# bastienjacquet/CudaDepthMapIntegration

Measured on AMD Instinct MI355X. Metric: Gvoxel-projections/s, higher is better.
Workload: dtype f64

## Files before the change

### cudadepthmapintegration_amd/build.py

```python
from __future__ import annotations

import os
import re
import shutil
import subprocess
from concurrent.futures import ThreadPoolExecutor

_HERE = os.path.dirname(os.path.abspath(__file__))
ROOT = os.path.dirname(_HERE)
CSRC = os.path.join(_HERE, "csrc")
OBJ_DIR = os.path.join(ROOT, "build", "obj")
LIB_PATH = os.path.join(CSRC, "libdmi_hip.so")

SOURCES = ["fusion_kernels.hip", "fusion_tile.hip", "fusion_classify.hip", "coloration_kernels.hip", "mesh_depth_render.hip", "grid_post.hip", "point_smooth.hip", "isosurface.hip", "isosurface_components.hip", "isosurface_smooth.hip", "isosurface_decimate.hip", "isosurface_holes.hip", "isosurface_support.hip", "depth_consistency.hip", "depth_speckle.hip", "depth_holes.hip", "depth_smooth.hip", "scene_bounds.hip", "depth_points.hip", "depth_points_thin.hip", "depth_points_radius.hip", "dmi_capi.hip", "dmi_capi_views.hip", "dmi_capi_fuse.hip", "dmi_capi_mesh.hip", "dmi_capi_color.hip", "dmi_capi_consistency.hip", "dmi_capi_speckle.hip", "dmi_capi_holes.hip", "dmi_capi_smooth.hip", "dmi_capi_bounds.hip", "dmi_capi_points_thin.hip", "dmi_capi_points_radius.hip", "view_set_kernels.hip", "dmi_capi_viewset.hip", "dmi_multi.hip", "host/recon_host.cpp", "host/vti_reader.cpp", "host/vtp_reader.cpp", "host/recon_cli.cpp", "host/color_cli.cpp", "host/dmi_host_capi.cpp"]
HEADERS = ["fusion_kernels.h", "view_records.h", "fusion_launch_rules.h", "fusion_device.h", "dmi_buffer.h", "dmi_depth_call.h", "dmi_mesh_stage.h", "dmi_context.h", "dmi_color_context.h", "coloration_kernels.h", "mesh_depth_render.h", "depth_consistency.h", "depth_speckle.h", "depth_speckle_rules.h", "depth_holes.h", "depth_holes_rules.h", "depth_smooth.h", "depth_smooth_rules.h", "union_find_device.h", "scene_bounds.h", "scene_bounds_rules.h", "depth_points.h", "depth_points_rules.h", "depth_points_thin.h", "depth_points_thin_rules.h", "depth_points_radius.h", "depth_points_radius_rules.h", "dmi_view_set.h", "view_set_kernels.h", "view_set_rules.h", "point_smooth_rules.h", "rounded_quotient.h", "fusion_tile_acc.inc", "isosurface_table.inc", os.path.join("host", "recon_host.h"),
           os.path.join("host", "vtk_xml_data.h"), os.path.join("host", "vti_reader.h"), os.path.join("host", "vtp_reader.h"),
           os.path.join("host", "recon_cli.h"), os.path.join("host", "color_cli.h"), os.path.join("host", "fan_triangulate.h"),
           os.path.join("..", "..", "include", "dmi.h"), os.path.join("..", "..", "include", "dmi_host.h")]
CLI_MAINS = ["recon_cli_main.cpp", "color_cli_main.cpp"]

COMMON_FLAGS = ["-O3", "-std=c++17", "-fPIC", "-ffp-contract=off", "-fno-fast-math", "-Wall", "-Wno-unused-function",
                "-Wno-inline-asm", "-Wno-pass-failed"]
HIP_FLAGS = ["--offload-arch=gfx950", "-mllvm", "-disable-promote-alloca-to-vector", "-Xoffload-linker", "--discard-all"]
OPTIONAL_LLVM_FLAGS = ["-amdgpu-use-amdgpu-trackers=1"]
# ... 83 lines not shown
        return True
    t = os.path.getmtime(target)
    return any(os.path.getmtime(d) > t for d in deps)


LIB_OVERRIDE = os.environ.get("DMI_LIB_OVERRIDE")
if LIB_OVERRIDE:
    LIB_PATH = os.path.abspath(LIB_OVERRIDE)


def source_digest(files=None) -> str:
    import hashlib

    h = hashlib.sha256()
    h.update(" ".join(COMMON_FLAGS + HIP_FLAGS).encode())
    if files is None:
        files = [os.path.join(CSRC, s) for s in _sources()] + _headers() + [os.path.join(CSRC, "host", m) for m in CLI_MAINS]
    for f in files:
        h.update(os.path.relpath(f, CSRC).encode())
        with open(f, "rb") as fh:
            h.update(fh.read())
    return h.hexdigest()


def _digest_path() -> str:
    return LIB_PATH + ".digest"


def needs_build() -> bool:
    if LIB_OVERRIDE:
        return False
    if not os.path.exists(LIB_PATH):
        return True
    if os.path.exists(_digest_path()):
        with open(_digest_path()) as fh:
            return fh.read().strip() != source_digest()
    deps = [os.path.join(CSRC, s) for s in _sources()] + _headers()
    return _stale(LIB_PATH, deps)


ACC_BASES = {8: 64, 7: 72, 6: 80, 5: 96}


def audit_accumulator_registers(asm_text: str) -> tuple[int, list[str]]:
    import re

    bad: list[str] = []
    checked = 0
    for body in re.split(r"\n(?=_ZN3dmi\S*fuse_tile_kernel\S*:)", asm_text):
        m = re.match(r"(_ZN3dmi\S*fuse_tile_kernelI\w+):", body)
        if not m:
            continue
        name = m.group(1)
        tpl = re.search(r"fuse_tile_kernelI\w\wLi(\d+)ELi(\d)ELi(\d)ELi(\d)ELi(\d)ELb([01])", name)
        tk, minw = int(tpl.group(1)), int(tpl.group(4))
        base = ACC_BASES.get(minw, 128)
        code = body[: body.find("s_endpgm")]
        in_asm = False
        scc_from_asm = False
        for line in code.splitlines():
            if "#ASMSTART" in line:
                in_asm = True
                continue
            if "#ASMEND" in line:
                in_asm = False
                continue
            op = line.split()[0] if line.split() else ""
            if in_asm:
                if op.startswith("s_and_saveexec"):
                    scc_from_asm = True
            elif op.startswith("s_"):
                if scc_from_asm and re.match(r"s_(cbranch_scc|cselect|cmov|addc|subb)", op):
                    bad.append(f"{name}: {op} reads the SCC an asm statement's s_and_saveexec_b64 wrote: {line.strip()}")
                if not re.match(r"s_(mov|movk|load|buffer_load|waitcnt|nop|branch|cbranch|cselect|cmov|getpc|setpc|swappc|sleep|barrier|endpgm)", op):
                    scc_from_asm = False
            elif line.rstrip().endswith(":") and not line.startswith((" ", "\t")):
                scc_from_asm = False
            if in_asm or not re.match(r"\s+(v_|global_|buffer_|ds_|scratch_|flat_)", line):
                continue
            regs = [int(x) for x in re.findall(r"\bv(\d+)\b", line)]
            for a, b in re.findall(r"\bv\[(\d+):(\d+)\]", line):
                regs += [int(a), int(b)]
            if any(r >= base for r in regs):
                bad.append(f"{name}: compiler instruction touches the accumulator file (base v{base}): {line.strip()}")
        d = re.search(r"\.amdhsa_kernel " + re.escape(name) + r"\b.*?\.amdhsa_next_free_vgpr (\d+)", asm_text, re.S)
        if not d:
            bad.append(f"{name}: no kernel descriptor found")
        elif int(d.group(1)) < base + 2 * tk:
            bad.append(f"{name}: descriptor allocates {d.group(1)} VGPRs, the accumulators need {base + 2 * tk}")
        checked += 1
    if checked == 0:
        bad.append("no fuse_tile_kernel instantiation found in the assembly")
    return checked, bad


def scratch_sizes(asm_text: str) -> dict:
    import re

    out = {}
    for m in re.finditer(r"\.amdhsa_kernel (_ZN3dmi\S*fuse_tile_kernel\S*)\b(.*?)\.end_amdhsa_kernel", asm_text, re.S):
        size = re.search(r"\.amdhsa_private_segment_fixed_size (\d+)", m.group(2))
        out[m.group(1)] = int(size.group(1)) if size else 0
    return out


def lds_sizes(asm_text: str) -> dict:
    out = {}
    for m in re.finditer(r"\.amdhsa_kernel (_ZN3dmi\S*fuse_tile_kernel\S*)\b(.*?)\.end_amdhsa_kernel", asm_text, re.S):
        size = re.search(r"\.amdhsa_group_segment_fixed_size (\d+)", m.group(2))
        out[m.group(1)] = int(size.group(1)) if size else 0
    return out


def wait_state_counts(asm_text: str) -> dict:
    import re

    out = {}
    for m in re.finditer(r"^(_ZN3dmi\S*fuse_tile_kernel\S*):.*?\.end_amdhsa_kernel", asm_text, re.S | re.M):
        out[m.group(1)] = len(re.findall(r"^\s*s_nop\b", m.group(0), re.M))
    return out


def _audit_digest() -> str:
    return source_digest([os.path.join(CSRC, "fusion_tile.hip")] + _headers())


def audit_is_current() -> bool:
    import json

    marker = os.path.join(OBJ_DIR, "acc_audit.json")
    try:
        with open(marker) as fh:
            return json.load(fh).get("digest") == _audit_digest()
    except (OSError, ValueError):
        return False


def run_accumulator_audit(verbose: bool = False) -> int:
    import json
    import tempfile

    hipcc = hipcc_path()
    with tempfile.TemporaryDirectory() as tmp:
        out = os.path.join(tmp, "fusion_tile.s")
        cmd = [hipcc] + COMMON_FLAGS + HIP_FLAGS + ["--cuda-device-only", "-S", os.path.join(CSRC, "fusion_tile.hip"), "-o", out]
        if verbose:
            print(" ".join(cmd), flush=True)
        subprocess.check_call(cmd)
        with open(out) as fh:
            text = fh.read()
    checked, bad = audit_accumulator_registers(text)
    scratch = scratch_sizes(text)
    nops = wait_state_counts(text)
    lds = lds_sizes(text)
    table = {}
    for name, size in scratch.items():
        m = re.search(r"fuse_tile_kernelI(\w)(\w)Li(\d+)ELi(\d)ELi(\d)ELi(\d)ELi(\d)ELb([01])ELb([01])ELb([01])ELb([01])ELb([01])(?:ELb([01]))?E", name)
        if not m:
            continue
        depth, grid, tk, wx, wy, minw, group, count, rot, genk, stay, win, zf = m.groups()
        key = f"depth={depth} grid={grid} tk={tk} waves={wx}x{wy} count={count} rot={rot} genk={genk} stay={stay} win={win} zf={zf or 0}"
        production = depth == "f" and count == "0" and genk == "0" and wx == "1" and wy == "1"
        limit = None if not production else ((16 if "-DDMI_TUNING" in COMMON_FLAGS else 0) if tk == "16" else 48)
        table[key] = {"scratch_bytes_per_lane": size, "production": production, "limit": limit, "s_nop": nops.get(name),
                      "lds_bytes_per_workgroup": lds.get(name, 0)}
        if limit is not None and size > limit:
            bad.append(f"{name}: {size} bytes of scratch memory per lane in a production instantiation (limit {limit})")
        waves_per_cu = 4 * (4 if tk == "16" else 5)
        if production and lds.get(name, 0) * waves_per_cu > 160 * 1024:
            bad.append(f"{name}: {lds[name]} bytes of LDS per one-wave workgroup: {waves_per_cu} of them do not fit a CU's 160 KB")
    if bad:
        raise RuntimeError("accumulator-register audit of fusion_tile.hip FAILED (a toolchain change broke the hidden "
                           "register file; results would be silently wrong):\n  " + "\n  ".join(bad[:20]))
    version = subprocess.run([hipcc, "--version"], capture_output=True, text=True).stdout.strip().splitlines()
    os.makedirs(OBJ_DIR, exist_ok=True)
    with open(os.path.join(OBJ_DIR, "acc_audit.json"), "w") as fh:
        json.dump({"instantiations": checked, "violations": 0, "hipcc": version[:2], "digest": _audit_digest(),
                   "scratch_bytes_per_lane": {"max": max(scratch.values()) if scratch else None,
                                              "instantiations_with_scratch": sum(1 for v in scratch.values() if v),
                                              "production_max": max([v["scratch_bytes_per_lane"] for v in table.values() if v["production"]] or [0])},
                   "instantiation_table": table}, fh, indent=1)
    if verbose:
        print(f"accumulator audit: {checked} fuse_tile_kernel instantiations clean ({version[0] if version else 'hipcc'})", flush=True)
    return checked


def _record(mode: str) -> None:
    import json
    import time

    try:
        os.makedirs(OBJ_DIR, exist_ok=True)
        with open(os.path.join(OBJ_DIR, "build_record.json"), "w") as fh:
            json.dump({"mode": mode, "library": os.path.relpath(LIB_PATH, ROOT), "digest": source_digest(), "time": time.time(),
                       "flags": COMMON_FLAGS + HIP_FLAGS}, fh)
    except OSError:
        pass


def build(force: bool = False, verbose: bool = False) -> str:
    if not force and not needs_build():
        _record("up_to_date: the library's digest file names the present sources and flags; nothing compiled")
        return LIB_PATH
    hipcc = hipcc_path()
    os.makedirs(OBJ_DIR, exist_ok=True)
    headers = _headers()
    digest = source_digest()
    if not force and os.path.exists(LIB_PATH) and os.path.exists(_digest_path()):
        srcs = [os.path.join(CSRC, s) for s in _sources()]
        if not any(_stale(_obj(s), [p] + headers) for s, p in zip(_sources(), srcs)):
# ... 67 lines not shown
```

### cudadepthmapintegration_amd/csrc/fusion_tile.hip

```cpp
#include <stdlib.h>

#include <algorithm>
#include <type_traits>

#include "fusion_kernels.h"
#include "fusion_device.h"

#ifndef DMI_T1_CHAINS
#define DMI_T1_CHAINS 4
#endif
#ifndef DMI_T1_COLUMN_CHAINS
#define DMI_T1_COLUMN_CHAINS 2
#endif
#if !defined(DMI_TUNING) && (defined(DMI_EXP_SKIP_WINDOW_VIEWS) || defined(DMI_EXP_SAME_REC) || defined(DMI_EXP_NO_WINDOW_LOADS) || \
                             defined(DMI_EXP_NO_LANE_MARGIN))
#error "a DMI_EXP_* switch that changes results was defined without DMI_TUNING"
#endif

namespace dmi {

int tile_shape_index(int variant);

namespace {

constexpr int kLX = 8, kLY = 8;
typedef unsigned long long mask_t;


#include "fusion_tile_acc.inc"

__device__ __forceinline__ void or_where(uint32_t &bits, mask_t m, uint32_t bit ) {
  mask_t saved;
  asm("s_and_saveexec_b64 %1, %2\n\tv_or_b32 %0, %3, %0\n\ts_mov_b64 exec, %1" : "+v"(bits), "=&s"(saved) : "s"(m), "s"(bit) : "scc");
}

__device__ __forceinline__ mask_t ballot(bool p) { return __builtin_amdgcn_ballot_w64(p); }

template <typename P>
__device__ __forceinline__ P launder(P p) {
  asm volatile("" : "+s"(p));
  return p;
}

__device__ __forceinline__ int pinned_word(int x) {
  asm volatile("" : "+v"(x));
  return __builtin_amdgcn_readfirstlane(x);
}
template <typename T>
__device__ __forceinline__ const T *pinned_ptr(const T *p) {
  const uintptr_t v = reinterpret_cast<uintptr_t>(p);
  const uint32_t lo = (uint32_t)pinned_word((int)(uint32_t)v), hi = (uint32_t)pinned_word((int)(uint32_t)(v >> 32));
  return reinterpret_cast<const T *>(((uintptr_t)hi << 32) | lo);
}
__device__ __forceinline__ double pinned(double x) {
  return __hiloint2double(pinned_word(__double2hiint(x)), pinned_word(__double2loint(x)));
}

__device__ __forceinline__ int cvt_saturating(double x) {
  int r;
  asm("v_cvt_i32_f64 %0, %1" : "=v"(r) : "v"(x));
  return r;
}

typedef float f32x2 __attribute__((ext_vector_type(2)));
__device__ __forceinline__ f32x2 pk_fma_lo0_vs(f32x2 a, f32x2 b, unsigned long long c_bits) {
  f32x2 d;
// ... 154 lines not shown
  static __device__ __forceinline__ raw_t load_at(__amdgpu_buffer_rsrc_t rsrc, unsigned byte_offset) {
    typedef unsigned int u32x2 __attribute__((ext_vector_type(2)));
    const u32x2 raw = __builtin_amdgcn_raw_buffer_load_b64(rsrc, (int)byte_offset, 0, 0);
    return __hiloint2double((int)raw.y, (int)raw.x);
  }
  static __device__ __forceinline__ void opaque(raw_t &d) { asm("" : "+v"(d)); }
  static __device__ __forceinline__ bool is_sentinel(raw_t d) { return d == -1.0; }
  static __device__ __forceinline__ raw_t sentinel() { return -1.0; }
  static __device__ __forceinline__ raw_t minus_inf() { return -__builtin_inf(); }
  static __device__ __forceinline__ double widen(raw_t d) { return d; }
};

template <typename DepthT>
__device__ __forceinline__ bool tile_exact(const FuseArgs *__restrict__ fa, int m, __amdgpu_buffer_rsrc_t rsrc, int i,
                                           int j, int k, double &val) {
  double g[12], rt[12], kk[12];
  const MapRec *maps = cload(&fa->maps);
#pragma unroll
  for (int q = 0; q < 12; ++q) {
    g[q] = cload(&fa->g[q]);
    rt[q] = cload(&maps[m].rt[q]);
    kk[q] = cload(&maps[m].k[q]);
  }
  const int W = cload(&fa->W), H = cload(&fa->H);
  const double gx = cload(&fa->ox) + (i + 0.5) * cload(&fa->sx);
  const double gy = cload(&fa->oy) + (j + 0.5) * cload(&fa->sy);
  const double gz = cload(&fa->oz) + ((k + cload(&fa->kz0)) + 0.5) * cload(&fa->sz);
  const double wx = row4(g + 0, gx, gy, gz);
  const double wy = row4(g + 4, gx, gy, gz);
  const double wz = row4(g + 8, gx, gy, gz);
  const double cx = row4(rt + 0, wx, wy, wz);
  const double cy = row4(rt + 4, wx, wy, wz);
  const double cz = row4(rt + 8, wx, wy, wz);
  const double hx = row4(kk + 0, cx, cy, cz);
  const double hy = row4(kk + 4, cx, cy, cz);
  const double hz = row4(kk + 8, cx, cy, cz);
  int px = 0, py = 0;
  if (!pixel_exact(hx, hy, hz, W, H, px, py)) return false;
  const typename DepthLoad<DepthT>::raw_t d = DepthLoad<DepthT>::load(rsrc, (unsigned)(W * py + px));
  if (DepthLoad<DepthT>::is_sentinel(d)) return false;
  val = ray_potential_values(cload(&fa->thick), cload(&fa->delta), cload(&fa->rho_pos), cload(&fa->rho_neg), cload(&fa->rho_zero),
                             cload(&fa->slope), cload(&fa->free_space), cz, DepthLoad<DepthT>::widen(d));
  return true;
}

constexpr int acc_base(int minw) { return minw >= 8 ? 64 : minw == 7 ? 72 : minw == 6 ? 80 : minw == 5 ? 96 : 128; }

template <typename DepthT, typename GridT, int TK, int WX, int WY, int MINW, int GROUP, bool COUNT, bool ROT = false, bool GENK = false,
          bool STAY = (WX * WY == 1), bool WIN = false, bool ZF = false>
__global__ __launch_bounds__(64 * WX * WY, MINW) void fuse_tile_kernel(const TileArgs a) {
  typedef DepthLoad<DepthT> DL;
  static_assert(!WIN || (DMI_TIER1 != 0 && !GENK && !COUNT && WX * WY == 1), "the window column is a tier-1 column without hit counters");
  static_assert(!ZF || !COUNT, "hit counters take every view singly");
  typedef const TileArgs __attribute__((address_space(4))) *kernarg_t;
  const kernarg_t ka = (kernarg_t)__builtin_amdgcn_kernarg_segment_ptr();
  (void)a;
#define KA(f) (ka->f)
#define KC(f) (launder(ka)->f)
#define KFRESH() launder(ka)
  constexpr int BASE = acc_base(MINW);
  constexpr int kGroup = GROUP;
  typedef double czvec __attribute__((ext_vector_type(GROUP)));
  typedef double czvec4 __attribute__((ext_vector_type(4)));
  const int first_map = KA(first_map);
  const int m_end = first_map + KA(n_maps);
  double delta = KA(delta), thick = KA(thick), free_space = KA(free_space), rho_pos = KA(rho_pos), slope = KA(slope);
  int keep_zero_adds = ZF ? 0 : (KA(behind_mask) == 0 ? 1 : 0);
  free_space = pinned(free_space), rho_pos = pinned(rho_pos);
  if constexpr (!ZF) keep_zero_adds = pinned_word(keep_zero_adds);
  asm volatile("" : "+v"(delta), "+v"(thick), "+v"(slope));
  unsigned vW = (unsigned)KA(W), vH = (unsigned)KA(H);
  asm("" : "+v"(vW));
  asm("" : "+v"(vH));
  [[maybe_unused]] const double Wd = pinned((double)KA(W));
  constexpr bool T1 = DMI_TIER1 != 0 && !GENK;
  [[maybe_unused]] const float Wf = __int_as_float(pinned_word(__float_as_int((float)KA(W))));
  [[maybe_unused]] const unsigned row_bytes = (unsigned)pinned_word((int)((unsigned)KA(W) * (unsigned)sizeof(DepthT)));
  [[maybe_unused]] unsigned pix_adj = ((unsigned)(KA(W) * (KA(H) / 2) + KA(W) / 2) - 0x400000u * (unsigned)KA(W)) * (unsigned)sizeof(DepthT) - 0x4B400000u;
  constexpr bool kConstantsInVgprs = TK >= 16;
  if constexpr (T1 && kConstantsInVgprs) asm volatile("" : "+v"(pix_adj));
  if constexpr (T1 && !kConstantsInVgprs) pix_adj = (unsigned)pinned_word((int)pix_adj);
  double tiny = 0x1p-20;
  asm volatile("" : "+v"(tiny));
  const int lane = threadIdx.x & 63;
  const int w = __builtin_amdgcn_readfirstlane(threadIdx.x >> 6);

  constexpr bool PERSIST = STAY && WX * WY == 1;
  const int b = blockIdx.x;
  int q = b >> 3;
  int helped = 0;
#define DMI_NEXT_BRICK \
  {                    \
    if (PERSIST)       \
      continue;        \
    else               \
      return;          \
  }
  for (;;) {
  const kernarg_t kb = KFRESH();
  typedef int i32x8 __attribute__((ext_vector_type(8)));
  const i32x8 head0 = *reinterpret_cast<const i32x8 __attribute__((address_space(4))) *>(kb);
  const i32x8 head1 = *(reinterpret_cast<const i32x8 __attribute__((address_space(4))) *>(kb) + 1);
  const int32_t *const p_order = kb->order, *const p_levels = kb->order_levels, *const p_n_order = kb->n_order;
  const int kflags = kb->flags;
  const int xq = (b + helped) & 7;
  if constexpr (PERSIST) {
// ... 619 lines not shown
    if constexpr (T1) {
      hx = __builtin_fma(cload(&rec->cpx), wxf,
                         __builtin_fma(cload(&rec->cpy), wyf, __builtin_fma(cload(&rec->cpz), wzf, cload(&rec->cp0))));
      hy = __builtin_fma(cload(&rec->cqx), wxf,
                         __builtin_fma(cload(&rec->cqy), wyf, __builtin_fma(cload(&rec->cqz), wzf, cload(&rec->cq0))));
      const float czf = (float)cz_first;
      H0.x = (float)hx;
      H0.y = (float)hy;
      C0.x = czf;
      const float hb = max_abs(H0.x, H0.y) + cload(&rec->t1_hspan);
      float e1 = cload(&rec->t1_e1);
      if (cload(&rec->t1_ok) == 2) e1 = t1_lane_margin<TK>(czf, cload(&rec->t1_dcz), hb, e1, cload(&rec->t1_b));
      C0.y = __builtin_fmaf(czf, cload(&rec->t1_c1), -__builtin_fmaf(hb, cload(&rec->t1_erel), e1));
      DH.x = cload(&rec->t1_dhx);
      DH.y = cload(&rec->t1_dhy);
      DC.x = cload(&rec->t1_dcz);
      DC.y = cload(&rec->t1_dthr);
      asm volatile("" : "+v"(DH), "+v"(DC));
    } else if constexpr (!ROT) {
      hx = __builtin_fma(cload(&rec->px), wx,
                         __builtin_fma(cload(&rec->py), wy, __builtin_fma(cload(&rec->pz), wz0, cload(&rec->p0))));
      hy = __builtin_fma(cload(&rec->qx), wx,
                         __builtin_fma(cload(&rec->qy), wy, __builtin_fma(cload(&rec->qz), wz0, cload(&rec->q0))));
    }
    [[maybe_unused]] const double dhx = T1 ? 0.0 : cload(&rec->dhx), dhy = T1 ? 0.0 : cload(&rec->dhy), errk = T1 ? 0.0 : cload(&rec->errk);
    [[maybe_unused]] double hz = 0, dhz = 0, errz = 0;
    if constexpr (GENK) {
      dhz = cload(&rec->dhz);
      errz = cload(&rec->errz);
      if constexpr (!ROT) {
        hz = __builtin_fma(cload(&rec->sx), wx, __builtin_fma(cload(&rec->sy), wy, __builtin_fma(cload(&rec->sz), wz0, cload(&rec->s0))));
        if (!lane_ok) hz = -__builtin_inf();
      }
    }

    [[maybe_unused]] auto rot_cz = [&](int kk) __attribute__((always_inline)) -> double {
      if (kk >= kcount) return -__builtin_inf();
      const kernarg_t kr = KFRESH();
      const TileMapRec *rr = kr->tile_maps + m;
      const czvec4 b = cload(reinterpret_cast<const czvec4 *>(kr->cz_table + (int64_t)(k0 + kk) * 4));
      const double wxk = (wx + b[0]) + kr->g[3], wyk = (wy + b[1]) + kr->g[7], wzk = (wz0 + b[2]) + kr->g[11];
      return ((cload(&rr->rz0) * wxk + cload(&rr->rz1) * wyk) + cload(&kr->maps[m].rt[10]) * wzk) + sz;
    };

    uint32_t undecided = 0;
    uint32_t und_kk = 0;
    uint32_t map_hits = 0;

    auto column = [&](auto interior_tag, auto surface_tag, auto free_tag) __attribute__((always_inline)) {
      constexpr bool INTERIOR = decltype(interior_tag)::value;
      constexpr bool FREEONLY = decltype(free_tag)::value;
      constexpr bool SURFACE = decltype(surface_tag)::value;
      constexpr bool UNMASKED = INTERIOR && !COUNT;
      [[maybe_unused]] int cxc = 0, cyc = 0;
      [[maybe_unused]] unsigned bias_x = 0, bias_y = 0;
      if constexpr (T1 && !INTERIOR) {
        cxc = KC(W) >> 1;
        cyc = KC(H) >> 1;
        bias_x = 0x4B400000u - (unsigned)cxc;
        bias_y = 0x4B400000u - (unsigned)cyc;
        if constexpr (kConstantsInVgprs) asm volatile("" : "+v"(bias_x), "+v"(bias_y));
      }
      constexpr bool VMAP = T1 && FREEONLY;
      const __amdgpu_buffer_rsrc_t rsrc =
          __builtin_amdgcn_make_buffer_rsrc(const_cast<void *>(cload(&rec->depth)), (short)0, KC(depth_bytes), 0x00020000);
      mask_t m_lane_ok = m_lane_ok_brick;
      asm volatile("" : "+s"(m_lane_ok));
      [[maybe_unused]] __amdgpu_buffer_rsrc_t vrsrc = rsrc;
      [[maybe_unused]] float v_c0 = 0.f, v_w8 = 0.f;
      [[maybe_unused]] int v_base = 0;
      if constexpr (VMAP) {
        vrsrc = __builtin_amdgcn_make_buffer_rsrc(const_cast<uint8_t *>(cload(&rec->valid)), (short)0, cload(&rec->vm_bytes), 0x00020000);
        v_c0 = cload(&rec->vm_c0);
        v_w8 = cload(&rec->vm_w8);
        v_base = cload(&rec->vm_base);
      }
  #pragma unroll
      for (int g0 = 0; g0 < TK; g0 += kGroup) {
        double czg[kGroup];
        typename DL::raw_t dg[kGroup];
        [[maybe_unused]] unsigned short vg[kGroup];
        if constexpr (!ROT && !(T1 && FREEONLY)) {
          const czvec ctg = cload(reinterpret_cast<const czvec *>(ct + g0));
  #pragma unroll
          for (int q = 0; q < kGroup; ++q) czg[q] = (sz + ctg[q]) + rz3;
          __builtin_amdgcn_sched_barrier(0);
        }
        if constexpr (ROT && T1 && !FREEONLY) {
          const double c20 = cload(&rec->rz0), c21 = cload(&rec->rz1), c22 = cload(&kv->maps[m].rt[10]);
  #pragma unroll
          for (int q = 0; q < kGroup; ++q) {
            const int kk = g0 + q;
            czg[q] = -__builtin_inf();
            if (kk < kcount) {
              const czvec4 b = cload(reinterpret_cast<const czvec4 *>(kv->cz_table + (int64_t)(k0 + kk) * 4));
              const double wxk = (wx + b[0]) + KA(g)[3], wyk = (wy + b[1]) + KA(g)[7], wzk = (wz0 + b[2]) + KA(g)[11];
              czg[q] = ((c20 * wxk + c21 * wyk) + c22 * wzk) + sz;
            }
          }
        }
        constexpr int kChain = T1 && TK >= 16 ? DMI_T1_COLUMN_CHAINS : 1;
        static_assert(kGroup % kChain == 0, "whole chains per group");
  #pragma unroll
        for (int q0 = 0; q0 < kGroup; q0 += kChain) {
        [[maybe_unused]] f32x2 rpm_c[kChain], rp_c[kChain];
        [[maybe_unused]] float mx_c[kChain], thr_c[kChain];
        if constexpr (T1) {
          f32x2 h[kChain], cth[kChain], rr[kChain], t[kChain];
          const unsigned long long magic2 = 0x4B4000004B400000ull;
  #pragma unroll
          for (int u = 0; u < kChain; ++u) {
            const int kk = g0 + q0 + u;
            cth[u] = kk > 0 ? ordered::pk_fma_s((unsigned long long)(unsigned)__float_as_int((float)kk), DC, C0) : C0;
          }
  #pragma unroll
          for (int u = 0; u < kChain; ++u) {
            const int kk = g0 + q0 + u;
            h[u] = kk > 0 ? ordered::pk_fma_s((unsigned long long)(unsigned)__float_as_int((float)kk), DH, H0) : H0;
          }
  #pragma unroll
          for (int u = 0; u < kChain; ++u) rr[u].x = ordered::rcp(cth[u].x);
  #pragma unroll
          for (int u = 0; u < kChain; ++u) rpm_c[u] = ordered::pk_fma_lo_s(h[u], rr[u], magic2);
  #pragma unroll
          for (int u = 0; u < kChain; ++u) rp_c[u] = ordered::pk_sub_s(rpm_c[u], magic2);
  #pragma unroll
          for (int u = 0; u < kChain; ++u) t[u] = ordered::pk_fnma_lo(rp_c[u], cth[u], h[u]);
  #pragma unroll
          for (int u = 0; u < kChain; ++u) {
            mx_c[u] = ordered::max_abs(t[u].x, t[u].y);
            thr_c[u] = cth[u].y;
          }
        }
  #pragma unroll
        for (int qc = 0; qc < kChain; ++qc) {
          const int q = q0 + qc;
          const int kk = g0 + q;
          if constexpr (!UNMASKED) dg[q] = DL::sentinel();
          if constexpr (T1) {
            const f32x2 rpm = rpm_c[qc], rp = rp_c[qc];
            unsigned pix;
            if constexpr (VMAP) {
              const float yt = __builtin_rintf(__builtin_fmaf(rp.y, 0.125f, v_c0));
              pix = (unsigned)(cvt_i32_f32(__builtin_fmaf(yt, v_w8, __builtin_fmaf(rp.x, 8.0f, rp.y))) + v_base);
            } else {
              pix = __umul24((unsigned)__float_as_int(rpm.y), row_bytes) +
                    scaled_column_bits<sizeof(DepthT)>(rp.x) + pix_adj;
            }
            const mask_t m_p1 = ballot(mx_c[qc] < thr_c[qc]);
            mask_t m_in, m_und;
            [[maybe_unused]] mask_t m_front = 0;
            if constexpr (INTERIOR) {
              m_in = m_p1 & m_lane_ok;
              m_und = m_lane_ok & ~m_p1;
            } else {
              m_front = ballot(!(czg[q] < 0.0));
              const unsigned px1 = (unsigned)__float_as_int(rpm.x) - bias_x, py1 = (unsigned)__float_as_int(rpm.y) - bias_y;
              m_in = m_front & m_p1 & ballot((unsigned)px1 < vW) & ballot((unsigned)py1 < vH);
              m_und = m_front & ~m_p1;
            }
            if (m_und) {
              const double kd = (double)kk;
              const double hxk = __builtin_fma(kd, cload(&rec->cdhx), hx), hyk = __builtin_fma(kd, cload(&rec->cdhy), hy);
              double cz2;
              if constexpr (FREEONLY)
                cz2 = ROT ? rot_cz(kk) : (sz + cload(ct + kk)) + rz3;
              else
                cz2 = czg[q];
              const double r0 = __builtin_amdgcn_rcp(cz2);
              const double e0 = __builtin_fma(-cz2, r0, 1.0);
              const double r = __builtin_fma(r0, e0, r0);
              const double ua2 = hxk * r, va2 = hyk * r;
              const double ru2 = __builtin_rint(ua2), rv2 = __builtin_rint(va2);
              const double fu = ua2 - ru2, fv = va2 - rv2;
              const double chk = __builtin_fma(cload(&rec->cerrk), r, __builtin_fmax(__builtin_fabs(fu), __builtin_fabs(fv)));
              const mask_t m_p2 = ballot(chk < 0.5) & ballot(__builtin_fabs(e0) < tiny) & m_und;
              unsigned pix2;
              if constexpr (VMAP) {
                const double yt2 = __builtin_rint(__builtin_fma(rv2, 0.125, (double)v_c0));
                pix2 = (unsigned)(cvt_saturating(__builtin_fma(yt2, (double)v_w8, __builtin_fma(ru2, 8.0, rv2))) + v_base);
              } else {
                pix2 = (unsigned)(cvt_saturating(__builtin_fma(rv2, Wd, ru2)) + (KC(W) * (KC(H) >> 1) + (KC(W) >> 1))) * (unsigned)sizeof(DepthT);
              }
              if (__builtin_amdgcn_inverse_ballot_w64(m_p2)) pix = pix2;
              if constexpr (INTERIOR) {
                m_in |= m_p2;
              } else {
                const int px2 = cvt_saturating(ru2) + cxc, py2 = cvt_saturating(rv2) + cyc;
                m_in |= m_p2 & ballot((unsigned)px2 < vW) & ballot((unsigned)py2 < vH);
              }
              m_und &= ~m_p2;
            }
            if constexpr (VMAP && UNMASKED) {
              vg[q] = __builtin_amdgcn_raw_buffer_load_b8(vrsrc, (int)pix, 0, 0);
              if (m_und) {
                or_where(undecided, m_und, 1u << kk);
                und_kk |= 1u << kk;
                if (__builtin_amdgcn_inverse_ballot_w64(m_und)) vg[q] = 0;
              }
            } else if constexpr (UNMASKED) {
              dg[q] = DL::load_at(rsrc, pix);
              if (m_und) {
                or_where(undecided, m_und, 1u << kk);
                und_kk |= 1u << kk;
                if (__builtin_amdgcn_inverse_ballot_w64(m_und)) dg[q] = SURFACE ? DL::minus_inf() : DL::sentinel();
              }
            } else {
              if (m_und) {
                or_where(undecided, m_und, 1u << kk);
                und_kk |= 1u << kk;
              }
              if (__builtin_amdgcn_inverse_ballot_w64(m_in)) dg[q] = DL::load_at(rsrc, pix);
            }
            continue;
          }
          if constexpr (ROT) {
            if (kk >= kcount) continue;
            const czvec4 b = cload(reinterpret_cast<const czvec4 *>(kv->cz_table + (int64_t)(k0 + kk) * 4));
// ... 15 lines not shown
              if constexpr (GENK) hz += dhz;
            }
          } else {
            if constexpr (GENK) {
              if (kk >= kcount) continue;
            }
            if (kk > 0) {
              hx += dhx;
              hy += dhy;
              if constexpr (GENK) hz += dhz;
            }
          }
          const double cz = czg[q];
          const double hdiv = GENK ? hz : cz;
          const double r0 = __builtin_amdgcn_rcp(hdiv);
          const double e0 = __builtin_fma(-hdiv, r0, 1.0);
          const double r = __builtin_fma(r0, e0, r0);
          const double ua = hx * r, va = hy * r;
          const double ru = __builtin_rint(ua), rv = __builtin_rint(va);
          const double fu = ua - ru, fv = va - rv;
          const double chk = __builtin_fma(errk, r, __builtin_fmax(__builtin_fabs(fu), __builtin_fabs(fv)));
          const mask_t m_proven = ballot(chk < 0.5) & ballot(__builtin_fabs(e0) < tiny);
          mask_t m_in, m_und;
          [[maybe_unused]] mask_t m_proven_front = ~0ull;
          if constexpr (INTERIOR) {
            m_in = m_proven & m_lane_ok;
            m_und = m_lane_ok & ~m_proven;
          } else {
            const mask_t m_front = GENK ? ballot(!(hz < -errz)) : ballot(!(cz < 0.0));
            if constexpr (GENK) m_proven_front = ballot(hz > errz);
            m_in = m_front & m_proven & m_proven_front;
            m_und = m_front & ~(m_proven & m_proven_front);
          }
          if constexpr (UNMASKED) {
            dg[q] = DL::load(rsrc, (unsigned)cvt_saturating(__builtin_fma(rv, Wd, ru)));
            if (m_und) {
              or_where(undecided, m_und, 1u << kk);
              und_kk |= 1u << kk;
              if (__builtin_amdgcn_inverse_ballot_w64(m_und)) dg[q] = SURFACE ? DL::minus_inf() : DL::sentinel();
            }
          } else {
            const int px = cvt_saturating(ru), py = cvt_saturating(rv);
            if constexpr (!INTERIOR)
              m_in &= ballot((unsigned)px < vW) & ballot((unsigned)py < vH);
            if (m_und) {
              or_where(undecided, m_und, 1u << kk);
              und_kk |= 1u << kk;
            }
            if (__builtin_amdgcn_inverse_ballot_w64(m_in))
              dg[q] = DL::load(rsrc, __umul24((unsigned)py, vW) + (unsigned)px);
          }
        }
        }
  #pragma unroll
        for (int q = 0; q < kGroup; ++q) {
          const int kk = g0 + q;
          if constexpr (VMAP) {
            static_assert(kValidByte == 10, "((1 << 10) - 1) << 20 == 0x3ff00000");
            unsigned one_or_zero_hi;
            asm("v_bfm_b32 %0, %1, 20" : "=v"(one_or_zero_hi) : "v"(__builtin_bit_cast(_Float16, vg[q])));
            acc_fma_vs<BASE, TK>(kk, __hiloint2double((int)one_or_zero_hi, 0), free_space);
            continue;
          }
          const typename DL::raw_t d = dg[q];
          if constexpr (ZF && !FREEONLY) {
            if constexpr (std::is_same<DepthT, double>::value) {
              if constexpr (SURFACE) acc_potential_all_f64<BASE, TK>(kk, d, czg[q], delta, thick, slope, free_space, rho_pos);
              else acc_potential_f64<BASE, TK>(kk, d, czg[q], delta, thick, slope, free_space, rho_pos);
            } else {
              if constexpr (SURFACE) acc_potential_all_f32<BASE, TK>(kk, d, czg[q], delta, thick, slope, free_space, rho_pos);
              else acc_potential_f32<BASE, TK>(kk, d, czg[q], delta, thick, slope, free_space, rho_pos);
            }
            continue;
          }
          const mask_t m_hit = SURFACE ? ~0ull : ballot(!DL::is_sentinel(d));
          if constexpr (FREEONLY) {
            acc_add_s<BASE, TK>(kk, m_hit, free_space);
            continue;
          }
          if (SURFACE || m_hit) {
            const double diff = czg[q] - DL::widen(d);
            const mask_t m_front_far = ballot(diff < -delta);
            const mask_t m_behind_far = ballot(diff > delta);
            acc_add_s<BASE, TK>(kk, m_hit & m_front_far, free_space);
            if (!SURFACE && keep_zero_adds) acc_add_zero<BASE, TK>(kk, m_hit & m_behind_far);
            const mask_t m_near = m_hit & ~(m_front_far | m_behind_far);
            {
              if (m_near) {
                const int rh = __double2hiint(rho_pos) ^ (__double2hiint(diff) & (int)0x80000000);
                const double near = __builtin_fabs(diff) > thick ? __hiloint2double(rh, __double2loint(rho_pos)) : slope * diff;
                acc_add_v<BASE, TK>(kk, m_near, near);
              }
            }
            if (COUNT) {
              nh[kk] += __builtin_amdgcn_inverse_ballot_w64(m_hit) ? 1u : 0u;
              map_hits += (uint32_t)__popcll(m_hit);
            }
          }
        }
      }
    };
    const bool interior = kcount == TK && (cbyte & 0x1fu) >= ((unsigned)MIXED_NAN_DEPTH << 2) && !(kv->flags & TILE_FLAG_NO_INTERIOR);
    if (interior) {
      if constexpr (!COUNT) {
        if ((cbyte & 0x1fu) == ((unsigned)MIXED_FREE_OR_NODEPTH << 2 | BRICK_MIXED))
          column(std::true_type{}, std::false_type{}, std::true_type{});
#ifndef DMI_EXP_NO_SURFACE_COLUMN
        else if ((cbyte & 0x1fu) == ((unsigned)MIXED_NEAR_SURFACE << 2 | BRICK_MIXED) && !keep_zero_adds)
          column(std::true_type{}, std::true_type{}, std::false_type{});
// ... 120 lines not shown
  constexpr bool one_wave = WX * WY == 1;
  constexpr bool rare = std::is_same<DepthT, double>::value || GENK;
  static_assert(!WIN || (one_wave && !rare), "window launches are production launches");
  const int per_round = 8 * a.xcd_run_wg;
  unsigned blocks = (unsigned)((a.super_x * a.super_y * a.super_z * 32 + 32 + per_round - 1) / per_round * per_round);
  const dim3 block(64 * WX * WY);
  const bool zf = a.behind_mask != 0 && !cfg.count_hits;
  if (WIN && !zf) return hipErrorInvalidValue;
  bool stay = true;
  if constexpr (one_wave && !rare) {
    const int64_t voxels = (int64_t)a.super_x * a.super_y * a.super_z * 32 * 64 * TK;
    stay = (cfg.variant & VAR_PERSISTENT_ALWAYS) ? true
           : (cfg.variant & VAR_PERSISTENT_NEVER) ? false
           : (cfg.variant & VAR_NO_BRICK_CLASSES) ? true
           : cfg.holes ? (a.n_maps >= 48 && voxels >= (int64_t(1) << 25))
                       : (a.n_maps >= kPersistentMinViews && voxels >= (int64_t(1) << 27));
  }
  auto launch = [&](auto kernel, bool persistent, auto which) {
    unsigned n = blocks;
    if (persistent && one_wave) {
      static const unsigned resident = resident_workgroups(kernel, 64);
      n = std::min(n, resident);
    }
    (void)which;
    hipLaunchKernelGGL(kernel, dim3(n), block, 0, s, a);
    return hipGetLastError();
  };
  typedef std::integral_constant<int, 0> counted_t;
  typedef std::integral_constant<int, 1> per_brick_t;
  typedef std::integral_constant<int, 2> persistent_t;
  typedef std::integral_constant<int, 3> general_t;
  if constexpr (!WIN) {
    if (cfg.count_hits) return launch(fuse_tile_kernel<DepthT, GridT, TK, WX, WY, MINW, GROUP, true, ROT, GENK>, true, counted_t{});
  }
  if constexpr (one_wave && !rare) {
    if (zf) {
      if (!stay) return launch(fuse_tile_kernel<DepthT, GridT, TK, WX, WY, MINW, GROUP, false, ROT, GENK, false, WIN, true>, false, per_brick_t{});
      return launch(fuse_tile_kernel<DepthT, GridT, TK, WX, WY, MINW, GROUP, false, ROT, GENK, true, WIN, true>, true, persistent_t{});
    }
  }
  if constexpr (!WIN) return launch(fuse_tile_kernel<DepthT, GridT, TK, WX, WY, MINW, GROUP, false, ROT, GENK>, true, general_t{});
  return hipErrorInvalidValue;
}

int effective_shape(int variant, bool depth_is_f64, bool rotated, bool general_k = false) {
  int shape = tile_shape_index(variant);
#ifndef DMI_TUNING
  shape = (shape == 1 || shape == 3 || shape == 4 || shape == 7) ? 7 : 0;
#endif
  if (general_k || depth_is_f64) return 0;
  return (rotated && shape != 7) ? 0 : shape;
}

template <typename DepthT, typename GridT, int TK, int MINW, bool ROT>
hipError_t launch_win(const TileArgs &a, const FuseConfig &cfg, hipStream_t s) {
  if constexpr (DMI_TIER1 != 0 && std::is_same<DepthT, float>::value)
    return launch_shape<DepthT, GridT, TK, 1, 1, MINW, 8, ROT, false, true>(a, cfg, s);
  else
    return hipErrorInvalidValue;
}

template <typename DepthT, typename GridT>
hipError_t launch_types(const TileArgs &a, const FuseConfig &cfg, hipStream_t s) {
  constexpr bool f32_depth = std::is_same<DepthT, float>::value;
  const int shape = effective_shape(cfg.variant, !f32_depth, a.rotated != 0, cfg.general_k != 0);
  const bool win = DMI_TIER1 != 0 && std::is_same<DepthT, float>::value && a.win_origin != nullptr && !cfg.count_hits && !cfg.general_k &&
                   a.behind_mask != 0;
#ifdef DMI_FAST_BUILD
  if (win) {
    if (shape == 7) return launch_win<DepthT, GridT, 8, 6, false>(a, cfg, s);
    return launch_win<DepthT, GridT, 16, 5, false>(a, cfg, s);
  }
  if constexpr (f32_depth) {
    if (shape == 7) return launch_shape<DepthT, GridT, 8, 1, 1, 6, 8>(a, cfg, s);
  }
  return launch_shape<DepthT, GridT, 16, 1, 1, 5, 8>(a, cfg, s);
#else
  if (cfg.general_k) {
    if (a.rotated) return launch_shape<DepthT, GridT, 16, 1, 1, 5, 8, true, true>(a, cfg, s);
    return launch_shape<DepthT, GridT, 16, 1, 1, 5, 8, false, true>(a, cfg, s);
  }
  if (a.rotated) {
    if (win) {
      if (shape == 7) return launch_win<DepthT, GridT, 8, 6, true>(a, cfg, s);
      return launch_win<DepthT, GridT, 16, 5, true>(a, cfg, s);
    }
    if constexpr (f32_depth) {
      if (shape == 7) return launch_shape<DepthT, GridT, 8, 1, 1, 6, 8, true>(a, cfg, s);
    }
    return launch_shape<DepthT, GridT, 16, 1, 1, 5, 8, true>(a, cfg, s);
  }
#ifdef DMI_TUNING
  if constexpr (std::is_same<DepthT, float>::value) {
    switch (shape) {
      case 1: return launch_shape<DepthT, GridT, 8, 2, 2, 6, 8>(a, cfg, s);
      case 2: return launch_shape<DepthT, GridT, 16, 2, 2, 5, 8>(a, cfg, s);
      case 3: return launch_shape<DepthT, GridT, 8, 2, 2, 6, 4>(a, cfg, s);
      case 4: return launch_shape<DepthT, GridT, 8, 2, 2, 7, 8>(a, cfg, s);
      case 5: return launch_shape<DepthT, GridT, 16, 2, 2, 5, 4>(a, cfg, s);
      case 6: return launch_shape<DepthT, GridT, 16, 2, 2, 6, 2>(a, cfg, s);
      default: break;
    }
  }
#endif
  if (win && (shape == 7 || shape == 0)) {
    if (shape == 7) return launch_win<DepthT, GridT, 8, 6, false>(a, cfg, s);
    return launch_win<DepthT, GridT, 16, 5, false>(a, cfg, s);
  }
  if constexpr (f32_depth) {
    if (shape == 7) return launch_shape<DepthT, GridT, 8, 1, 1, 6, 8>(a, cfg, s);
  }
  return launch_shape<DepthT, GridT, 16, 1, 1, 5, 8>(a, cfg, s);
#endif
}

}

int tile_shape_index(int variant) { return (variant & VAR_TILE_SHAPE_MASK) >> VAR_TILE_SHAPE_SHIFT; }

TileShape tile_shape(int variant, bool depth_is_f64, bool rotated, bool general_k) {
  switch (effective_shape(variant, depth_is_f64, rotated, general_k)) {
    case 0: return TileShape{16, 1, 1};
    case 7: return TileShape{8, 1, 1};
    case 1:
    case 3:
    case 4: return TileShape{8, 2, 2};
    default: return TileShape{16, 2, 2};
  }
}

#ifdef DMI_TUNING
__global__ __launch_bounds__(256) void remap_classes_kernel(uint8_t *classes, int64_t n, uint32_t table) {
  for (int64_t i = (int64_t)blockIdx.x * blockDim.x + threadIdx.x; i < n; i += (int64_t)gridDim.x * blockDim.x) {
    const uint8_t b = classes[i];
    classes[i] = (uint8_t)((table >> (8 * (b & 3))) & 0xff);
  }
}
#endif

hipError_t launch_fuse_tiled(const TileArgs &a, const MapRec *maps_dev, const FuseConfig &cfg, const PyramidDesc &pyramid,
                             uint8_t *order_scratch, uint8_t *coarse_classes, hipEvent_t before_main_kernel,
                             hipStream_t stream) {
  if (a.n_maps <= 0) return hipSuccess;
  hipError_t e = hipSuccess;
  if (cfg.variant & VAR_NO_BRICK_CLASSES) {
    const int64_t entries = a.rotated ? a.kpad : (int64_t)a.kpad * a.n_maps;
    hipLaunchKernelGGL(launch_tables_kernel, dim3((unsigned)std::min<int64_t>((entries + 255) / 256, 4096)), dim3(256), 0, stream, a, maps_dev);
    e = hipGetLastError();
    if (e != hipSuccess) return e;
  }
  if (!(cfg.variant & VAR_NO_BRICK_CLASSES)) {
    const TileShape sh = tile_shape(cfg.variant, cfg.depth_is_f64 != 0, a.rotated != 0, cfg.general_k != 0);
    e = launch_classify_bricks(a, maps_dev, pyramid, sh.tk, const_cast<uint8_t *>(a.classes), coarse_classes, cfg.general_k, stream);
    if (e != hipSuccess) return e;
    e = launch_window_origins(a, maps_dev, sh.tk, const_cast<uint8_t *>(a.classes), cfg.general_k, stream);
    if (e != hipSuccess) return e;
#ifdef DMI_TUNING
    if (const char *env = getenv("DMI_DEBUG_CLASS_REMAP")) {
      const int64_t n = (int64_t)a.wbricks_x * a.wbricks_y * a.bricks_z * (int64_t)a.class_pitch;
      hipLaunchKernelGGL(remap_classes_kernel, dim3(4096), dim3(256), 0, stream, const_cast<uint8_t *>(a.classes), n,
                         (uint32_t)strtoul(env, nullptr, 0));
    }
#endif
    if (a.order) {
      e = launch_order_bricks(a, sh.wx, sh.wy, order_scratch, const_cast<int *>(a.order), const_cast<int *>(a.n_order), stream);
// ... 19 lines not shown
```

Baseline: 3193.

## Issue a whole 16-voxel column of depth loads per group, forming c.z late

For TK=16 tier-1 kernels on f32 depth, the load group grows from 8 to 16 so more depth loads are in flight before use. To keep register pressure in check, the per-voxel camera z values are no longer precomputed for the whole group. They are recomputed on demand in phase A and loaded in batches of four in phase B. The build audit regexes now accept a two-digit GROUP template argument. This risks higher VGPR use or spills and adds redundant c.z arithmetic in return for more memory-level parallelism.

```diff
diff --git a/cudadepthmapintegration_amd/build.py b/cudadepthmapintegration_amd/build.py
--- a/cudadepthmapintegration_amd/build.py
+++ b/cudadepthmapintegration_amd/build.py
@@ -159,7 +159,7 @@
         if not m:
             continue
         name = m.group(1)
-        tpl = re.search(r"fuse_tile_kernelI\w\wLi(\d+)ELi(\d)ELi(\d)ELi(\d)ELi(\d)ELb([01])", name)
+        tpl = re.search(r"fuse_tile_kernelI\w\wLi(\d+)ELi(\d)ELi(\d)ELi(\d)ELi(\d+)ELb([01])", name)
         tk, minw = int(tpl.group(1)), int(tpl.group(4))
         base = ACC_BASES.get(minw, 128)
         code = body[: body.find("s_endpgm")]
@@ -262,7 +262,7 @@
     lds = lds_sizes(text)
     table = {}
     for name, size in scratch.items():
-        m = re.search(r"fuse_tile_kernelI(\w)(\w)Li(\d+)ELi(\d)ELi(\d)ELi(\d)ELi(\d)ELb([01])ELb([01])ELb([01])ELb([01])ELb([01])(?:ELb([01]))?E", name)
+        m = re.search(r"fuse_tile_kernelI(\w)(\w)Li(\d+)ELi(\d)ELi(\d)ELi(\d)ELi(\d+)ELb([01])ELb([01])ELb([01])ELb([01])ELb([01])(?:ELb([01]))?E", name)
         if not m:
             continue
         depth, grid, tk, wx, wy, minw, group, count, rot, genk, stay, win, zf = m.groups()
diff --git a/cudadepthmapintegration_amd/csrc/fusion_tile.hip b/cudadepthmapintegration_amd/csrc/fusion_tile.hip
--- a/cudadepthmapintegration_amd/csrc/fusion_tile.hip
+++ b/cudadepthmapintegration_amd/csrc/fusion_tile.hip
@@ -12,6 +12,10 @@
 #ifndef DMI_T1_COLUMN_CHAINS
 #define DMI_T1_COLUMN_CHAINS 2
 #endif
+#ifndef DMI_COLUMN_LOAD_GROUP
+#define DMI_COLUMN_LOAD_GROUP 16
+#endif
+static_assert(DMI_COLUMN_LOAD_GROUP == 16 || DMI_COLUMN_LOAD_GROUP == 8, "a whole 16-voxel column or half of one");
 #if !defined(DMI_TUNING) && (defined(DMI_EXP_SKIP_WINDOW_VIEWS) || defined(DMI_EXP_SAME_REC) || defined(DMI_EXP_NO_WINDOW_LOADS) || \
                              defined(DMI_EXP_NO_LANE_MARGIN))
 #error "a DMI_EXP_* switch that changes results was defined without DMI_TUNING"
@@ -272,6 +276,8 @@
   typedef DepthLoad<DepthT> DL;
   static_assert(!WIN || (DMI_TIER1 != 0 && !GENK && !COUNT && WX * WY == 1), "the window column is a tier-1 column without hit counters");
   static_assert(!ZF || !COUNT, "hit counters take every view singly");
+  static_assert(GROUP <= 8 || (DMI_TIER1 != 0 && !GENK && sizeof(DepthT) == 4),
+                "more than eight loads in flight: tier-1 columns on f32 depth tables (c.z is formed in phase B, a raw depth is one register)");
   typedef const TileArgs __attribute__((address_space(4))) *kernarg_t;
   const kernarg_t ka = (kernarg_t)__builtin_amdgcn_kernarg_segment_ptr();
   (void)a;
@@ -997,6 +1003,11 @@
       constexpr bool FREEONLY = decltype(free_tag)::value;
       constexpr bool SURFACE = decltype(surface_tag)::value;
       constexpr bool UNMASKED = INTERIOR && !COUNT;
+      constexpr bool kCzLate = kGroup > 8;
+      [[maybe_unused]] auto cz_on_demand = [&](int kk) __attribute__((always_inline)) -> double {
+        if constexpr (ROT) return rot_cz(kk);
+        else return (sz + cload(ct + kk)) + rz3;
+      };
       [[maybe_unused]] int cxc = 0, cyc = 0;
       [[maybe_unused]] unsigned bias_x = 0, bias_y = 0;
       if constexpr (T1 && !INTERIOR) {
@@ -1025,13 +1036,13 @@
         double czg[kGroup];
         typename DL::raw_t dg[kGroup];
         [[maybe_unused]] unsigned short vg[kGroup];
-        if constexpr (!ROT && !(T1 && FREEONLY)) {
+        if constexpr (!kCzLate && !ROT && !(T1 && FREEONLY)) {
           const czvec ctg = cload(reinterpret_cast<const czvec *>(ct + g0));
   #pragma unroll
           for (int q = 0; q < kGroup; ++q) czg[q] = (sz + ctg[q]) + rz3;
           __builtin_amdgcn_sched_barrier(0);
         }
-        if constexpr (ROT && T1 && !FREEONLY) {
+        if constexpr (!kCzLate && ROT && T1 && !FREEONLY) {
           const double c20 = cload(&rec->rz0), c21 = cload(&rec->rz1), c22 = cload(&kv->maps[m].rt[10]);
   #pragma unroll
           for (int q = 0; q < kGroup; ++q) {
@@ -1099,7 +1110,10 @@
               m_in = m_p1 & m_lane_ok;
               m_und = m_lane_ok & ~m_p1;
             } else {
-              m_front = ballot(!(czg[q] < 0.0));
+              double cz1;
+              if constexpr (kCzLate) cz1 = cz_on_demand(kk);
+              else cz1 = czg[q];
+              m_front = ballot(!(cz1 < 0.0));
               const unsigned px1 = (unsigned)__float_as_int(rpm.x) - bias_x, py1 = (unsigned)__float_as_int(rpm.y) - bias_y;
               m_in = m_front & m_p1 & ballot((unsigned)px1 < vW) & ballot((unsigned)py1 < vH);
               m_und = m_front & ~m_p1;
@@ -1108,7 +1122,9 @@
               const double kd = (double)kk;
               const double hxk = __builtin_fma(kd, cload(&rec->cdhx), hx), hyk = __builtin_fma(kd, cload(&rec->cdhy), hy);
               double cz2;
-              if constexpr (FREEONLY)
+              if constexpr (kCzLate)
+                cz2 = cz_on_demand(kk);
+              else if constexpr (FREEONLY)
                 cz2 = ROT ? rot_cz(kk) : (sz + cload(ct + kk)) + rz3;
               else
                 cz2 = czg[q];
@@ -1230,9 +1246,32 @@
           }
         }
         }
+        constexpr int kCzBatch = 4;
+        static_assert(!kCzLate || kGroup % kCzBatch == 0, "whole batches per group");
+        [[maybe_unused]] double c20 = 0, c21 = 0, c22 = 0;
+        if constexpr (kCzLate && ROT && !FREEONLY) c20 = cload(&rec->rz0), c21 = cload(&rec->rz1), c22 = cload(&kv->maps[m].rt[10]);
   #pragma unroll
         for (int q = 0; q < kGroup; ++q) {
           const int kk = g0 + q;
+          if constexpr (kCzLate && !FREEONLY) {
+            if (q % kCzBatch == 0) {
+              if constexpr (!ROT) {
+                const czvec4 ctb = cload(reinterpret_cast<const czvec4 *>(ct + kk));
+  #pragma unroll
+                for (int u = 0; u < kCzBatch; ++u) czg[q + u] = (sz + ctb[u]) + rz3;
+              } else {
+  #pragma unroll
+                for (int u = 0; u < kCzBatch; ++u) {
+                  czg[q + u] = -__builtin_inf();
+                  if (kk + u < kcount) {
+                    const czvec4 b = cload(reinterpret_cast<const czvec4 *>(kv->cz_table + (int64_t)(k0 + kk + u) * 4));
+                    const double wxk = (wx + b[0]) + KA(g)[3], wyk = (wy + b[1]) + KA(g)[7], wzk = (wz0 + b[2]) + KA(g)[11];
+                    czg[q + u] = ((c20 * wxk + c21 * wyk) + c22 * wzk) + sz;
+                  }
+                }
+              }
+            }
+          }
           if constexpr (VMAP) {
             static_assert(kValidByte == 10, "((1 << 10) - 1) << 20 == 0x3ff00000");
             unsigned one_or_zero_hi;
@@ -1459,10 +1498,15 @@
   return (rotated && shape != 7) ? 0 : shape;
 }
 
+template <typename DepthT, int TK>
+constexpr int column_load_group() {
+  return (TK == 16 && DMI_TIER1 != 0 && std::is_same<DepthT, float>::value) ? DMI_COLUMN_LOAD_GROUP : 8;
+}
+
 template <typename DepthT, typename GridT, int TK, int MINW, bool ROT>
 hipError_t launch_win(const TileArgs &a, const FuseConfig &cfg, hipStream_t s) {
   if constexpr (DMI_TIER1 != 0 && std::is_same<DepthT, float>::value)
-    return launch_shape<DepthT, GridT, TK, 1, 1, MINW, 8, ROT, false, true>(a, cfg, s);
+    return launch_shape<DepthT, GridT, TK, 1, 1, MINW, column_load_group<DepthT, TK>(), ROT, false, true>(a, cfg, s);
   else
     return hipErrorInvalidValue;
 }
@@ -1481,7 +1525,7 @@
   if constexpr (f32_depth) {
     if (shape == 7) return launch_shape<DepthT, GridT, 8, 1, 1, 6, 8>(a, cfg, s);
   }
-  return launch_shape<DepthT, GridT, 16, 1, 1, 5, 8>(a, cfg, s);
+  return launch_shape<DepthT, GridT, 16, 1, 1, 5, column_load_group<DepthT, 16>()>(a, cfg, s);
 #else
   if (cfg.general_k) {
     if (a.rotated) return launch_shape<DepthT, GridT, 16, 1, 1, 5, 8, true, true>(a, cfg, s);
@@ -1495,7 +1539,7 @@
     if constexpr (f32_depth) {
       if (shape == 7) return launch_shape<DepthT, GridT, 8, 1, 1, 6, 8, true>(a, cfg, s);
     }
-    return launch_shape<DepthT, GridT, 16, 1, 1, 5, 8, true>(a, cfg, s);
+    return launch_shape<DepthT, GridT, 16, 1, 1, 5, column_load_group<DepthT, 16>(), true>(a, cfg, s);
   }
 #ifdef DMI_TUNING
   if constexpr (std::is_same<DepthT, float>::value) {
@@ -1517,7 +1561,7 @@
   if constexpr (f32_depth) {
     if (shape == 7) return launch_shape<DepthT, GridT, 8, 1, 1, 6, 8>(a, cfg, s);
   }
-  return launch_shape<DepthT, GridT, 16, 1, 1, 5, 8>(a, cfg, s);
+  return launch_shape<DepthT, GridT, 16, 1, 1, 5, column_load_group<DepthT, 16>()>(a, cfg, s);
 #endif
 }
 
```

Result: no change. 3186 (-0.2%).
